# fjdf/slaMEM

Measured on AMD Instinct MI355X. Metric: MEMs/sec (and queries/sec) on 100 Mbp ref x 10 M 150 bp queries, l=20, higher is better.
Workload: dtype u32; 1 GPU; synthetic 100000000 bp reference (splitmix64 seed 42) x 10000000 reads/GPU of 150 bp, 2% substitutions, 50% reverse-complemented, -b -l 20; ref_len=100000000, reads_total=10000000, read_len=150, min_len=20, both_strands=True, parallelism=query shards x1, one GPU, no replication

## Files before the change

### include/slamem_hip.h

```cpp
#ifndef SLAMEM_HIP_H
#define SLAMEM_HIP_H

#include <stddef.h>
#include <stdint.h>

#ifdef __cplusplus
extern "C" {
#endif

#define SLAMEM_ABI_VERSION 4

enum {
    SLAMEM_OK = 0,
    SLAMEM_ERR_ARG = 1,
    SLAMEM_ERR_HIP = 2,
    SLAMEM_ERR_NOMEM = 3,
    SLAMEM_ERR_CAPACITY = 4,
    SLAMEM_ERR_FORMAT = 5,
    SLAMEM_ERR_IO = 6,
    SLAMEM_ERR_NO_DEVICE = 7
};

typedef struct slamem_index slamem_index;

// ... 69 lines not shown
    uint64_t positions;
    uint64_t enum_jobs;
    uint64_t prefilter_probes;
    uint64_t prefilter_query_loads;
    uint64_t prefilter_items;
    uint64_t items;
    uint64_t survivors;
    uint64_t mems;
    uint64_t overflow_records;
    uint64_t valid;
    uint64_t dir_sa_lines;
    uint64_t dir_group_loads;
    uint64_t dir_rec_lines;
    uint64_t dir_letters;
    uint64_t jump_lines;
    uint64_t skip_group_loads;
    uint64_t skip_probe_lines;
    uint64_t skip_attempts;
    uint64_t skips;
    uint64_t enum_row_steps;
    uint64_t enum_levels;
    uint64_t enum_wave_us;
    uint64_t state_lane_trips[11];
    uint64_t state_wave_trips[11];
    uint64_t seed_windows;
    uint64_t seed_compares;
    uint64_t seed_letter_masks;
    uint64_t seed_mems;
    uint64_t seed_strands_left;
    uint64_t seed_reads;
    uint64_t seed_query_bytes;
    uint64_t seed_left_why[7];
    uint64_t seed_once_reads;
} slamem_search_stats;

int slamem_abi_version(void);
const char *slamem_strerror(int code);
const char *slamem_last_error_message(void);
int slamem_device_count(int *count_out);
int slamem_device_warmup(int device);
int slamem_device_pci_bus_id(int device, char *out, int out_bytes);
int slamem_device_mem_info(int device, uint64_t *free_out, uint64_t *total_out);
int slamem_get_timings(slamem_timings *out);
int slamem_reset_timings(void);
int slamem_search_stats_enable(int on);
int slamem_get_search_stats(slamem_search_stats *out);
int slamem_get_search_clock(double *us_to_empty_list, double *us_tail, double *us_wave_sum);

int slamem_index_build(const char *text_host, uint32_t n, int device, slamem_index **out);
int slamem_index_build_device(const void *text_dev, uint32_t n, int device, void *stream, slamem_index **out);
int slamem_index_build_layout(const char *text_host, uint32_t n, int device, int layout, slamem_index **out);
int slamem_index_build_device_layout(const void *text_dev, uint32_t n, int device, void *stream, int layout,
                                     slamem_index **out);
int slamem_index_build_bytes(uint32_t n, int layout, uint64_t *arena_bytes_out, uint64_t *peak_bytes_out);
int slamem_index_free(slamem_index *idx);
int slamem_index_get_info(const slamem_index *idx, slamem_index_info *out);

int slamem_index_arena(const slamem_index *idx, void **arena_dev_out, uint64_t *bytes_out);
int slamem_index_export(const slamem_index *idx, void *dst_dev, uint64_t dst_bytes, void *stream);
int slamem_index_attach(void *arena_dev, uint64_t bytes, int device, slamem_index **out);
int slamem_index_adopt_arena(slamem_index *idx);
int slamem_index_save(const slamem_index *idx, const char *path);
int slamem_index_load(const char *path, int device, slamem_index **out);
int slamem_index_validate_header(const void *header, uint64_t header_bytes, uint64_t available_bytes);

enum {
// ... 190 lines not shown
```

### slamem_amd/capi.py

```python
from __future__ import annotations

import ctypes as C
import os

_HERE = os.path.dirname(os.path.abspath(__file__))
LIB_PATH = os.environ.get("SLAMEM_HIP_LIB") or os.path.join(_HERE, "csrc", "libslamem_hip.so")
SYNTH_PATH = os.path.join(_HERE, "csrc", "libslamem_synth.so")

SLAMEM_OK = 0
SLAMEM_ERR_ARG = 1
SLAMEM_ERR_HIP = 2
SLAMEM_ERR_NOMEM = 3
SLAMEM_ERR_CAPACITY = 4
SLAMEM_ERR_FORMAT = 5
SLAMEM_ERR_IO = 6
SLAMEM_ERR_NO_DEVICE = 7

ARRAY_SA, ARRAY_BWT, ARRAY_LCP, ARRAY_PSV, ARRAY_NSV = range(5)
LAYOUT_AUTO, LAYOUT_FULL, LAYOUT_COMPACT = 0, 1, 2

ABI_SYMBOLS = (
    "slamem_abi_version", "slamem_strerror", "slamem_last_error_message", "slamem_device_count",
    "slamem_get_timings", "slamem_reset_timings", "slamem_device_warmup", "slamem_device_pci_bus_id",
    "slamem_index_build", "slamem_index_build_device", "slamem_index_build_layout", "slamem_index_build_device_layout",
# ... 38 lines not shown
    _fields_ = [("text_length", C.c_uint32), ("bwt_size", C.c_uint32), ("num_n_rows", C.c_uint32),
                ("dollar_row", C.c_uint32), ("max_lcp", C.c_uint32), ("sort_rounds", C.c_uint32),
                ("arena_bytes", C.c_uint64), ("device", C.c_int32), ("owns_arena", C.c_int32),
                ("filter_k", C.c_uint32), ("layout", C.c_uint32), ("seed_k", C.c_uint32), ("reserved1", C.c_uint32)]


class SslcpStats(C.Structure):
    _fields_ = [("num_samples", C.c_uint64), ("num_oversized_lcp", C.c_uint64), ("sum_lcp", C.c_int64),
                ("max_lcp", C.c_uint32), ("pad", C.c_uint32), ("num_oversized_links", C.c_uint64),
                ("sum_link_distance", C.c_uint64), ("max_link_distance", C.c_uint64)]


class Timings(C.Structure):
    _fields_ = [("build_total_ms", C.c_float), ("build_pack_ms", C.c_float), ("build_sort_ms", C.c_float),
                ("build_bwt_ms", C.c_float), ("build_lcp_ms", C.c_float), ("build_links_ms", C.c_float),
                ("search_kernel_ms", C.c_float), ("search_total_ms", C.c_float),
                ("search_launches", C.c_uint64), ("search_kernel_ms_sum", C.c_double),
                ("prefilter_ms", C.c_float), ("k8_ms", C.c_float), ("prefilter_ms_sum", C.c_double),
                ("k8_ms_sum", C.c_double), ("seed_ms", C.c_float), ("mum_filter_ms", C.c_float), ("seed_ms_sum", C.c_double)]

    def as_dict(self):
        return {k: getattr(self, k) for k, _ in self._fields_}


class SearchStats(C.Structure):
    _fields_ = [(k, C.c_uint64) for k in (
        "fm_lines_top", "fm_lines_bottom", "rec_lines_fail", "rec_lines_pend", "rec_lines_flush", "query_loads",
        "lane_trips", "wave_trips", "positions", "enum_jobs", "prefilter_probes", "prefilter_query_loads",
        "prefilter_items", "items", "survivors", "mems", "overflow_records", "valid", "dir_sa_lines", "dir_group_loads",
        "dir_rec_lines", "dir_letters", "jump_lines", "skip_group_loads", "skip_probe_lines", "skip_attempts", "skips",
        "enum_row_steps", "enum_levels", "enum_wave_us")] + [("state_lane_trips", C.c_uint64 * 11),
                                                               ("state_wave_trips", C.c_uint64 * 11)] + [
        (k, C.c_uint64) for k in ("seed_windows", "seed_compares", "seed_letter_masks", "seed_mems", "seed_strands_left",
                                  "seed_reads", "seed_query_bytes")] + [("seed_left_why", C.c_uint64 * 7), ("seed_once_reads", C.c_uint64)]

    def as_dict(self):
        return {k: (list(getattr(self, k)) if (k.startswith("state_") or k == "seed_left_why") else int(getattr(self, k))) for k, _ in self._fields_}


_LIB = None
_SYNTH = None


def _declare(L):
    vp, u32, u64, i32 = C.c_void_p, C.c_uint32, C.c_uint64, C.c_int
    L.slamem_abi_version.restype = i32
    L.slamem_strerror.restype = C.c_char_p
    L.slamem_strerror.argtypes = [i32]
    L.slamem_last_error_message.restype = C.c_char_p
    L.slamem_device_count.argtypes = [C.POINTER(i32)]
    L.slamem_device_pci_bus_id.argtypes = [i32, C.c_char_p, i32]
    L.slamem_get_timings.argtypes = [C.POINTER(Timings)]
    L.slamem_index_build.argtypes = [C.c_char_p, u32, i32, C.POINTER(vp)]
    L.slamem_index_build_device.argtypes = [vp, u32, i32, vp, C.POINTER(vp)]
    L.slamem_index_build_layout.argtypes = [C.c_char_p, u32, i32, i32, C.POINTER(vp)]
    L.slamem_index_build_device_layout.argtypes = [vp, u32, i32, vp, i32, C.POINTER(vp)]
    L.slamem_index_build_bytes.argtypes = [u32, i32, C.POINTER(u64), C.POINTER(u64)]
    L.slamem_device_mem_info.argtypes = [i32, C.POINTER(u64), C.POINTER(u64)]
    L.slamem_index_free.argtypes = [vp]
    L.slamem_index_get_info.argtypes = [vp, C.POINTER(IndexInfo)]
    L.slamem_index_arena.argtypes = [vp, C.POINTER(vp), C.POINTER(u64)]
    L.slamem_index_export.argtypes = [vp, vp, u64, vp]
    L.slamem_index_attach.argtypes = [vp, u64, i32, C.POINTER(vp)]
    L.slamem_index_adopt_arena.argtypes = [vp]
    L.slamem_index_save.argtypes = [vp, C.c_char_p]
    L.slamem_index_load.argtypes = [C.c_char_p, i32, C.POINTER(vp)]
    L.slamem_index_validate_header.argtypes = [vp, u64, u64]
    L.slamem_search_stats_enable.argtypes = [i32]
    L.slamem_get_search_stats.argtypes = [C.POINTER(SearchStats)]
    L.slamem_get_search_clock.argtypes = [C.POINTER(C.c_double), C.POINTER(C.c_double), C.POINTER(C.c_double)]
# ... 126 lines not shown
```

### slamem_amd/csrc/mem_search.hip

```cpp
#include "common.h"
#include "prims.h"

#include <atomic>
#include <type_traits>
#include <new>
#include <stdlib.h>
#include <string.h>

namespace slamem {

struct Blk {
    uint4 a;
    uint4 b;
    uint4 c;
    uint4 d;
};

__device__ __forceinline__ uint64_t u64_of(uint32_t lo, uint32_t hi) { return ((uint64_t)hi << 32) | lo; }

__device__ __forceinline__ Blk load_blk(const FMBlock* __restrict__ fm, uint32_t bi) {
    const uint4* p = reinterpret_cast<const uint4*>(fm + bi);
    Blk k;
    k.a = p[0]; k.b = p[1]; k.c = p[2]; k.d = p[3];
    return k;
// ... 938 lines not shown
                    aoff = 0; boff = 0;
                    done = msz < L;
                }
                if (done) {
                    if (gl == 0u) A.defer.pool[segabs] = k - kbase;
                    busy = false;
                }
            }
        }
    }
#ifdef SLAMEM_DIAG_TRIPS
    if (lane == 0u) { atomicMax(A.defer.njobs + 11, dg_steps); atomicAdd(A.defer.njobs + 12, dg_steps); atomicAdd(A.defer.njobs + 13, dg_busy); }
#endif
}

__global__ void __launch_bounds__(256) k_defer_prefix(SearchArgs A) {
    const uint32_t n = *A.defer.nlist;
    for (uint32_t i = blockIdx.x * blockDim.x + threadIdx.x; i < n; i += gridDim.x * blockDim.x) {
        const uint2 e = A.defer.list[i];
        uint32_t* c = A.defer.pool + e.y;
        const uint32_t jobs = c[0], own = c[1];
        uint32_t run = 0;
        for (uint32_t s2 = 0; s2 < jobs; s2++) { const uint32_t v = c[2u + s2]; c[2u + s2] = run; run += v; }
        c[2u + jobs] = run;
        A.block_counts[e.x] = own + run;
    }
}

enum : uint32_t {
    SC_FM_TOP = 0, SC_FM_BOT, SC_REC_FAIL_LINES, SC_REC_PEND_LINES, SC_REC_FLUSH_LINES, SC_QUERY_LOADS, SC_LANE_TRIPS,
    SC_WAVE_TRIPS, SC_POSITIONS, SC_ENUM_JOBS, SC_ENUM_ROW_STEPS, SC_PF_PROBES, SC_PF_QUERY_LOADS, SC_PF_ITEMS,
    SC_DIR_SA, SC_DIR_GROUPS, SC_DIR_RECS, SC_DIR_QLOADS, SC_DIR_LETTERS, SC_JUMP_LINES,
    SC_SKIP_GROUPS, SC_SKIP_QLOADS, SC_SKIP_PROBES, SC_SKIP_OK, SC_T_FIRST, SC_T_DRAIN, SC_T_LAST, SC_T_WAVE_SUM, SC_ENUM_LEVELS, SC_T_ENUM_SUM, SC_STATE_TRIPS , SC_STATE_WAVES = SC_STATE_TRIPS + 11 ,
    SC_SEED_WINDOWS = SC_STATE_WAVES + 11, SC_SEED_COMPARES, SC_SEED_NMASKS, SC_SEED_MEMS, SC_SEED_LEFT, SC_SEED_READS, SC_SEED_QBYTES, SC_SEED_WHY , SC_SEED_ONCE = SC_SEED_WHY + 7, SC_COUNT
};
template <bool kStats>
__device__ __forceinline__ void stat_flush(unsigned long long* dst, uint32_t v) {
    if (!kStats) return;
    for (int o = 32; o > 0; o >>= 1) v += __shfl_down(v, o);
    if ((threadIdx.x & 63u) == 0u && v) atomicAdd(dst, (unsigned long long)v);
}

template <uint32_t kLanes>
__global__ void __launch_bounds__(256) k_pack_queries(SearchArgs A, bool long_only) {
    __shared__ uint8_t lut[512];
    for (uint32_t i = threadIdx.x; i < 256u; i += 256u) {
        uint32_t c = ascii_code_q(i);
        lut[i] = (uint8_t)c;
        lut[256u + i] = (uint8_t)(c >= 2u ? 7u - c : c);
    }
    __syncthreads();
    const uint32_t sub = threadIdx.x & (kLanes - 1u);
    const uint64_t count = long_only ? A.num_items : (A.work_ids ? (uint64_t)*A.work_count : A.num_items);
    const uint64_t stride = ((uint64_t)gridDim.x * blockDim.x) / kLanes;
    for (uint64_t e = ((uint64_t)blockIdx.x * blockDim.x + threadIdx.x) / kLanes; e < count; e += stride) {
    const uint64_t item = (!long_only && A.work_ids) ? (uint64_t)A.work_ids[e] : e;
    ItemDesc d;
    uint64_t pk_word;
    if (A.implicit_items) {
        if (!long_only && A.item_alive && A.item_alive[item] == 0) continue;
        d = item_of(A, item); pk_word = item_pk_of(A, item, d);
    }
    else {
        uint4 dv = *reinterpret_cast<const uint4*>(A.items + item);
        pk_word = A.item_pk[item];
        asm volatile("" : "+v"(dv.x), "+v"(dv.y), "+v"(dv.z), "+v"(dv.w), "+v"(pk_word));
        d.base = u64_of(dv.x, dv.y); d.len = dv.z; d.slice_rev = dv.w;
    }
// ... 1076 lines not shown
        unsigned long long smask[2 * R];
    };
    uint32_t flags;
    uint32_t pad[3];
};

__device__ __forceinline__ void wave_sync() {
    __builtin_amdgcn_fence(__ATOMIC_RELEASE, "wavefront");
    __builtin_amdgcn_wave_barrier();
    __builtin_amdgcn_fence(__ATOMIC_ACQUIRE, "wavefront");
}
__device__ __forceinline__ uint64_t funnel64(uint64_t lo, uint64_t hi, uint32_t sh) { return (lo >> sh) | ((hi << 1) << (63u - sh)); }
__device__ __forceinline__ uint64_t bits_below(int x) {
    const int c = x < 0 ? 0 : x > 64 ? 64 : x;
    return c == 0 ? 0ull : (~0ull >> (64 - c));
}
__device__ __forceinline__ uint64_t bits_range(int lo, int hi) { return bits_below(hi) & ~bits_below(lo); }
__device__ __forceinline__ uint32_t sel4(const uint4& v, uint32_t a) {
    const uint32_t lo = (a & 1u) ? v.y : v.x, hi = (a & 1u) ? v.w : v.z;
    return (a & 2u) ? hi : lo;
}
__device__ __forceinline__ uint32_t sel12(const uint4& b0, const uint4& b1, const uint4& b2, uint32_t e) {
    const uint32_t a = e & 3u, x0 = sel4(b0, a), x1 = sel4(b1, a), x2 = sel4(b2, a);
    return e < 4u ? x0 : e < 8u ? x1 : x2;
}
__device__ __forceinline__ uint32_t byte_tops(uint32_t m) {
    const uint32_t y = m >> 7;
    return (y | (y >> 7) | (y >> 14) | (y >> 21)) & 0xFu;
}

#ifndef SLAMEM_SEED_WAVES
#define SLAMEM_SEED_WAVES 1
#endif
template <bool kStats, uint32_t NW, uint32_t R>
__global__ void __launch_bounds__(256, SLAMEM_SEED_WAVES) k_seed_mems(SearchArgs A, uint8_t* __restrict__ alive) {
    constexpr uint32_t kMaxLen = 64u * NW;
    static_assert(R <= 32u && R * NW <= 128u, "a flag word holds a bit per read; the planes step runs in at most two passes");
    __shared__ SeedWave<NW, R> lds[4];
    const IndexView& ix = A.ix;
    const uint32_t lane = threadIdx.x & 63u, wv = threadIdx.x >> 6;
    SeedWave<NW, R>& S = lds[wv];
    const uint32_t strands = A.strands, k = ix.seed_k, L = A.min_len, s = L - k + 1u;
    const uint32_t kmask = (1u << k) - 1u;
    const uint64_t r0 = ((uint64_t)blockIdx.x * 4u + wv) * R;
    if (r0 >= (uint64_t)A.num_queries) return;
    const uint32_t nr = (uint64_t)A.num_queries - r0 < R ? (uint32_t)((uint64_t)A.num_queries - r0) : R;
    const unsigned long long below = (1ull << lane) - 1ull;
    const int64_t ulast = (int64_t)text_units(ix.n) - 1;
    uint32_t n_win = 0, n_cmp = 0, n_nm = 0, n_mem = 0;

    const uint64_t off = lane <= nr ? A.offsets[r0 + lane] : 0ull;
    constexpr uint32_t kRawChunks = R * NW * 4u + 1u, kSpecIters = (kRawChunks + 63u) / 64u;
#ifndef SLAMEM_SEED_NO_SPEC
    constexpr bool kSpec = kSpecIters <= 5u;
#else
    constexpr bool kSpec = false;
#endif
    uint4 sv[kSpec ? kSpecIters : 1u];
    uint64_t g0 = 0, len0 = 0;
    bool spec = false;
    if (kSpec) {
        const uint64_t o0 = A.offsets[0], o1 = A.offsets[1], o_end = A.offsets[A.num_queries];
        len0 = o1 - o0;
        g0 = o0 + r0 * len0;
        const uint64_t g1 = g0 + (uint64_t)nr * len0;
        spec = len0 != 0ull && len0 <= (uint64_t)kMaxLen && g1 <= o_end;
        const uint32_t gn = spec ? (uint32_t)(((g1 - 1u) >> 4) - (g0 >> 4) + 1u) : 0u;
        const uint4* src = reinterpret_cast<const uint4*>(A.qwords) + (g0 >> 4);
#pragma unroll
        for (uint32_t j = 0; j < kSpecIters; j++) {
            const uint32_t c = lane + 64u * j;
            sv[j] = c < gn ? src[c] : make_uint4(0, 0, 0, 0);
        }
    }
    const uint64_t offn = __shfl_down(off, 1);
    if (kSpec) spec = spec && __ballot(lane <= nr && off != g0 + (uint64_t)lane * len0) == 0ull;
    uint32_t len = 0, nwin = 0;
// ... 241 lines not shown
            njobs = njobs0;
        }
    };
    auto lookups = [&](uint32_t round) {
        const uint32_t step = round == 0u ? mstep : 1u;
        uint32_t cnt = 0;
        const uint32_t per = 64u >> lg_slots, wi = lane & ((1u << lg_slots) - 1u);
        const uint32_t wmod = wi - mstep * ((wi * (65536u / mstep + 1u)) >> 16);
        for (uint32_t r = 0;; r += per) {
            if (r < nr) {
                const uint32_t rr = r + (lane >> lg_slots);
                const uint32_t nw = (rr >= nr || ((S.flags >> rr) & 1u)) ? 0u : S.nwin[rr];
                const bool pred = wi < nw && (round == 0u ? wmod == 0u : wmod != 0u && ((S.expl[rr] >> wi) & 1ull) == 0ull);
                const unsigned long long pm = __ballot(pred);
                if (pred) S.ring[cnt + (uint32_t)__popcll(pm & below)] = (uint16_t)((rr << 8) | wi);
                cnt += (uint32_t)__popcll(pm);
            }
            const bool last = r >= nr;
            if (cnt >= 64u || (last && cnt != 0u)) {
                wave_sync();
                const bool act = lane < cnt;
                const uint32_t ent = act ? S.ring[lane] : 0u;
                const uint32_t over = lane + 64u < cnt ? S.ring[lane + 64u] : 0u;
                wave_sync();
                if (lane + 64u < cnt) S.ring[lane] = (uint16_t)over;
                cnt = cnt > 64u ? cnt - 64u : 0u;
                trip(ent, act, step);
            }
            if (last) break;
        }
        wave_sync();
    };

    auto compares = [&](uint32_t round) {
        const bool mark = round == 0u && mstep > 1u;
        const uint32_t ms = mstep * s;
        const uint32_t gone = S.flags;
        for (uint32_t jb = 0; jb < njobs; jb += 64u) {
            const bool listed = jb + lane < njobs;
            const uint32_t p = listed ? S.job_p[jb + lane] : 0u, xx = listed ? S.job_x[jb + lane] : 0u;
            const uint32_t os = xx & 0x7FFFu, st = (xx >> 15) & 1u, jr = xx >> 16;
            const bool has = listed && ((gone >> jr) & 1u) == 0u;
            const uint32_t Lj = S.len[jr];
            const int64_t d = (int64_t)p - (int64_t)os;
            const int64_t u0 = d >> 6;
            const uint32_t sh = (uint32_t)(d & 63);
            bool is_mem = false;
            uint32_t key = 0, ref = 0, sig = 0;
            if (has) {
                constexpr int NU = (int)NW + 1;
                int64_t ui[NU];
#pragma unroll
                for (int i = 0; i < NU; i++) { const int64_t u = u0 + i; ui[i] = u < 0 ? 0 : u > ulast ? ulast : u; }
                const uint4* T = reinterpret_cast<const uint4*>(ix.tpl);
                uint4 tu[NU], tx[NU];
#pragma unroll
                for (int i = 0; i < NU; i++) { tu[i] = T[2 * ui[i]]; tx[i] = T[2 * ui[i] + 1]; }
                uint64_t uq[NU], nu[NU];
                uint32_t anyn = 0;
#pragma unroll
                for (int i = 0; i < NU; i++) { nu[i] = u64_of(tx[i].x, tx[i].y); uq[i] = u64_of(tx[i].z, tx[i].w); anyn |= (tx[i].x | tx[i].y); }
                if (kStats && anyn) n_nm++;
                const uint64_t* R0 = S.pl[jr][st][0];
                const uint64_t* R1 = S.pl[jr][st][1];
                uint64_t mm[NW];
#pragma unroll
                for (int w = 0; w < (int)NW; w++)
                    mm[w] = (funnel64(u64_of(tu[w].x, tu[w].y), u64_of(tu[w + 1].x, tu[w + 1].y), sh) ^ R0[w]) |
                            (funnel64(u64_of(tu[w].z, tu[w].w), u64_of(tu[w + 1].z, tu[w + 1].w), sh) ^ R1[w]) | funnel64(nu[w], nu[w + 1], sh);
                if (hasn) {
                    const uint64_t* PN = S.pn[jr];
                    if (st == 0u) {
#pragma unroll
                        for (int w = 0; w < (int)NW; w++) mm[w] |= PN[w];
                    } else {
                        const uint32_t shn = kMaxLen - Lj, qn = shn >> 6, rn = shn & 63u;
#pragma unroll
                        for (int w = 0; w < (int)NW; w++) {
                            const uint32_t x = (uint32_t)w + qn;
                            const uint64_t lo64 = x < NW ? __brevll(PN[NW - 1u - x]) : 0ull, hi64 = x + 1u < NW ? __brevll(PN[NW - 2u - x]) : 0ull;
                            mm[w] |= funnel64(lo64, hi64, rn);
                        }
                    }
                }
                const int lo = d < 0 ? (int)(-d) : 0;
                const int64_t room = (int64_t)ix.n - d;
                const int hi = room < (int64_t)Lj ? (int)room : (int)Lj;
#pragma unroll
                for (int w = 0; w < (int)NW; w++) mm[w] |= ~bits_range(lo - 64 * w, hi - 64 * w);
                uint32_t a = 0, b = kMaxLen;
                bool broken = false;
#pragma unroll
                for (int w = 0; w < (int)NW; w++) {
                    const uint64_t lw = mm[w] & bits_range(0, (int)os - 64 * w);
                    if (lw) a = 64u * w + 64u - (uint32_t)__clzll((long long)lw);
                    if (mm[w] & bits_range((int)os - 64 * w, (int)(os + k) - 64 * w)) broken = true;
                }
#pragma unroll
                for (int w = (int)NW - 1; w >= 0; w--) {
                    const uint64_t hw = mm[w] & ~bits_range(0, (int)(os + k) - 64 * w);
                    if (hw) b = 64u * w + (uint32_t)__ffsll((unsigned long long)hw) - 1u;
                }
                const uint32_t af = st ? Lj - b : a, bf = st ? Lj - a : b, of = st ? Lj - k - os : os;
                bool owner;
                if (round == 0u) owner = !(of >= ms && of - ms >= af);
                else {
                    const uint32_t oa = (af + ms - 1u) / ms * ms;
                    owner = !(mstep > 1u && oa + k <= bf) && !(of >= s && of - s >= af);
                }
                if (broken) {
                    atomicOr(&S.flags, 1u << jr);
                    if (kStats) atomicAdd(A.stats + SC_SEED_WHY + 4u, 1ull);
                }
                else if (owner && b - a >= L && (strands == 2u || st == 0u)) {
                    is_mem = true; key = (a << 16) | (b - a); ref = (uint32_t)(d + (int64_t)a);
                    if (!anyn && b + kSigLetters <= kMaxLen && d + (int64_t)b + (int64_t)kSigLetters <= (int64_t)ix.n) {
                        const uint32_t wb = b >> 6, sb = b & 63u;
                        uint64_t l0 = 0, h0 = 0, l1 = 0, h1 = 0;
#pragma unroll
                        for (int w = 0; w < (int)NW; w++) {
                            const uint64_t t0 = funnel64(u64_of(tu[w].x, tu[w].y), u64_of(tu[w + 1].x, tu[w + 1].y), sh);
                            const uint64_t t1 = funnel64(u64_of(tu[w].z, tu[w].w), u64_of(tu[w + 1].z, tu[w + 1].w), sh);
                            if ((uint32_t)w == wb) { l0 = t0; l1 = t1; }
                            if ((uint32_t)w == wb + 1u) { h0 = t0; h1 = t1; }
                        }
                        sig = kSigKnown | ((uint32_t)funnel64(l0, h0, sb) & kSigMask) | (((uint32_t)funnel64(l1, h1, sb) & kSigMask) << kSigLetters);
                    }
                }
                if (mark && !broken && bf >= af + k) {
                    uint64_t uqs[NW];
#pragma unroll
                    for (int w = 0; w < (int)NW; w++) uqs[w] = funnel64(uq[w], uq[w + 1], sh);
                    unsigned long long done = 0ull;
                    for (uint32_t wi = (af + s - 1u) / s, wl = (bf - k) / s; wi <= wl; wi++) {
                        const uint32_t x = st ? Lj - k - wi * s : wi * s;
                        uint64_t word = 0ull;
#pragma unroll
                        for (int w = 0; w < (int)NW; w++) word = (x >> 6) == (uint32_t)w ? uqs[w] : word;
                        if ((word >> (x & 63u)) & 1ull) done |= 1ull << wi;
                    }
                    if (done) atomicOr(&S.expl[jr], done);
                }
            }
            if (kStats) {
                const uint32_t nh = (uint32_t)__popcll(__ballot(has));
                n_cmp += nh;
                if (mark && lane == 0u) atomicAdd(A.stats + SC_SEED_ONCE, (unsigned long long)nh);
            }
            const unsigned long long mb = __ballot(is_mem);
            if (is_mem) {
                const uint32_t at = nmems + (uint32_t)__popcll(mb & below);
                if (at < SeedWave<NW, R>::kMems) { S.mem_key[at] = key; S.mem_ref[at] = ref; S.mem_sig[at] = sig | ((2u * jr + st) << 25); }
                else { atomicOr(&S.flags, 1u << jr); if (kStats) atomicAdd(A.stats + SC_SEED_WHY + 5u, 1ull); }
            }
            nmems += (uint32_t)__popcll(mb);
        }
        wave_sync();
    };

    for (uint32_t round = 0; round < (mstep > 1u ? 2u : 1u); round++) {
        njobs = 0;
        lookups(round);
        compares(round);
    }
    };
    if (wave_hasn) search(std::true_type{}); else search(std::false_type{});
    {
        if (nmems > SeedWave<NW, R>::kMems) nmems = SeedWave<NW, R>::kMems;

        const uint32_t g0 = (uint32_t)(r0 * strands);
        auto rank_of = [&](uint32_t mi, uint32_t key, uint32_t g, uint32_t& rank, uint32_t& cnt, bool& tie) {
            rank = 0; cnt = 0; tie = false;
            for (uint32_t t2 = 0; t2 < nmems; t2++) {
                const uint32_t kk = S.mem_key[t2], gg = S.mem_sig[t2] >> 25;
                const bool same = gg == g;
                cnt += same ? 1u : 0u;
                rank += (same && kk > key) ? 1u : 0u;
                tie = tie || (same && kk == key && t2 != mi);
            }
        };
        auto tie_rank = [&](uint32_t mi, uint32_t key, uint32_t myref, uint32_t g, uint32_t sig, uint32_t& rank) -> bool {
            const uint32_t a = key >> 16, b = a + (key & 0xFFFFu);
            bool child = false;
            for (uint32_t t2 = 0; t2 < nmems; t2++) {
                const uint32_t kk = S.mem_key[t2], a2 = kk >> 16, b2 = a2 + (kk & 0xFFFFu);
                child = child || ((S.mem_sig[t2] >> 25) == g && kk != key && a2 <= a && b2 > b);
            }
            const uint32_t jr = g >> 1, st = g & 1u;
            uint32_t qb = 0;
            if (child) qb = (uint32_t)((S.pl[jr][st][0][b >> 6] >> (b & 63u)) & 1ull) | ((uint32_t)((S.pl[jr][st][1][b >> 6] >> (b & 63u)) & 1ull) << 1);
            auto letter = [&](uint32_t sg, uint32_t t) { return ((sg >> t) & 1u) | (((sg >> (t + kSigLetters)) & 1u) << 1); };
            const bool rows = ix.prec != nullptr;
            const uint32_t my_side = child && letter(sig, 0u) > qb ? 1u : 0u;
            bool bad = (sig & kSigKnown) == 0u && (child || !rows);
            for (uint32_t t2 = 0; t2 < nmems; t2++) {
                const uint32_t so = S.mem_sig[t2];
// ... 58 lines not shown
                    bool tie;
                    rank_of(mi, key, g, rank, cnt, tie);
                    const bool bad = has && tie && tie_rank(mi, key, ref, g, S.mem_sig[mi], rank);
                    if (!pass) { if (bad) atomicOr(&S.flags, 1u << (g >> 1)); }
                    else if (has) emit_mem(fl, key, ref, g, rank, cnt);
                }
                wave_sync();
            }
        }
    }
    wave_sync();
    const uint32_t fl = S.flags | wflags;
    {
        const bool isleft = lane < nr * strands && ((fl >> (strands == 2u ? lane >> 1 : lane)) & 1u) != 0u;
        if (lane < nr * strands) alive[r0 * strands + lane] = isleft ? 1 : 0;
        const unsigned long long lm = __ballot(isleft);
        if (lm != 0ull) {
            unsigned int at = 0;
            if (lane == 0u) at = atomicAdd(A.seed_left_count, (unsigned int)__popcll(lm));
            at = (unsigned int)__builtin_amdgcn_readfirstlane((int)at);
            if (isleft) A.seed_left_ids[at + (uint32_t)__popcll(lm & below)] = (uint32_t)(r0 * strands + lane);
        }
    }
    if (kStats) {
        stat_flush<kStats>(A.stats + SC_SEED_NMASKS, n_nm);
        stat_flush<kStats>(A.stats + SC_SEED_MEMS, n_mem);
        if (lane == 0u) {
            atomicAdd(A.stats + SC_SEED_WINDOWS, (unsigned long long)n_win);
            atomicAdd(A.stats + SC_SEED_COMPARES, (unsigned long long)n_cmp);
            atomicAdd(A.stats + SC_SEED_READS, (unsigned long long)nr);
            atomicAdd(A.stats + SC_SEED_QBYTES, (unsigned long long)(__builtin_amdgcn_readlane((int)(uint32_t)off, (int)nr) - __builtin_amdgcn_readlane((int)(uint32_t)off, 0)));
            atomicAdd(A.stats + SC_SEED_LEFT, (unsigned long long)(strands * (uint32_t)__popc(fl)));
            atomicAdd(A.stats + SC_SEED_WHY + 0u, (unsigned long long)__popc(wflags));
        }
    }
}

__global__ void __launch_bounds__(256) k_place_inline(const RawRow* __restrict__ inl, uint64_t stride, const uint32_t* __restrict__ counts,
                                                      const uint64_t* __restrict__ item_off, uint64_t nitems,
                                                      const uint32_t* __restrict__ sa, uint64_t capacity,
                                                      slamem_mem* __restrict__ out, const uint8_t* __restrict__ inline_valid) {
    uint64_t g = (uint64_t)blockIdx.x * blockDim.x + threadIdx.x;
    if (g >= nitems) return;
    uint32_t cnt = counts[g];
    uint64_t off = item_off[g];
    uint32_t iv = inline_valid ? inline_valid[g] : 0u;
    asm volatile("" : "+v"(cnt), "+v"(off), "+v"(iv));
    if (cnt > kInlineMems) cnt = kInlineMems;
    if (iv && cnt > iv - 1u) cnt = iv - 1u;
    if (cnt == 0u) return;
    static_assert(kInlineMems == 4, "k_place_inline is written for four inline slots");
    const RawRow* in = inl + g;
    const RawRow none = {0u, 0u, 0x80000000u};
    RawRow r0 = in[0], r1 = none, r2 = none, r3 = none;
    if (cnt > 1u) r1 = in[stride];
    if (cnt > 2u) r2 = in[2u * stride];
    if (cnt > 3u) r3 = in[3u * stride];
    asm volatile("" : "+v"(r0.row), "+v"(r0.pos), "+v"(r0.len), "+v"(r1.row), "+v"(r1.pos), "+v"(r1.len));
    asm volatile("" : "+v"(r2.row), "+v"(r2.pos), "+v"(r2.len), "+v"(r3.row), "+v"(r3.pos), "+v"(r3.len));
    uint32_t p0 = r0.row, p1 = r1.row, p2 = r2.row, p3 = r3.row;
    if (!(r0.len >> 31)) p0 = sa[r0.row];
    if (cnt > 1u && !(r1.len >> 31)) p1 = sa[r1.row];
    if (cnt > 2u && !(r2.len >> 31)) p2 = sa[r2.row];
    if (cnt > 3u && !(r3.len >> 31)) p3 = sa[r3.row];
    asm volatile("" : "+v"(p0), "+v"(p1), "+v"(p2), "+v"(p3));
    if (off < capacity) out[off] = slamem_mem{p0, r0.pos, r0.len & 0x7FFFFFFFu};
// ... 503 lines not shown

int SearchJob::prep(hipStream_t stream) {
    SLAMEM_HIP(hipSetDevice(idx->device));
    char* ws = static_cast<char*>(workspace_dev);
    unsigned long long* d_total = reinterpret_cast<unsigned long long*>(ws + w.off_total);
    uint32_t* d_counts = reinterpret_cast<uint32_t*>(ws + w.off_counts);
    prefiltered = false; timed_k8 = false; launched = true; seeded = false; rawkey_marked = false;
    (void)hipEventRecord(ev[0], stream);
    if (nitems && (match_type != 1 || mam_v3)) {
        static const bool use_filter = [] { const char* v = getenv("SLAMEM_KFILTER"); return !(v && atoi(v) == 0); }();
        seeded = seed_path;
        if (seeded) {
            uint8_t* d_alive = reinterpret_cast<uint8_t*>(ws + w.off_alive);
            if (mems_capacity && !A.skip_w && !want_stats && enum_chunks()) {
                STEP(hipMemsetAsync(ws + w.off_rawkey, 0xFF, mems_capacity * sizeof(RawKey), stream), "memset");
                rawkey_marked = true;
            }
            STEP(hipMemsetAsync(d_counts, 0, nitems * 4, stream), "memset");
            STEP(hipMemsetAsync(A.item_attempt, 0, nitems, stream), "memset");
            {
                const char* v = getenv("SLAMEM_SEED_STEP");
                A.seed_step = v && atoi(v) >= 1 && atoi(v) <= 6 ? (uint32_t)atoi(v) : 0u;
            }
            uint32_t* d_ids = reinterpret_cast<uint32_t*>(ws + w.off_workids);
            uint32_t* d_nwork = reinterpret_cast<uint32_t*>(d_total) + 8;
            A.seed_left_ids = d_ids;
            A.seed_left_count = d_nwork;
            A.seed_long_flag = reinterpret_cast<unsigned int*>(d_total) + 3;
            A.seed_wide = reinterpret_cast<unsigned int*>(d_total) + 4;
            seed_words_avg = query_bytes > (uint64_t)num_queries * kSeedMaxLenMid ? 6u : query_bytes > (uint64_t)num_queries * kSeedMaxLen ? 4u : 3u;
            const uint32_t hint = __atomic_load_n(&idx->seed_words_hint, __ATOMIC_RELAXED);
            seed_words = seed_words_avg > hint ? seed_words_avg : hint;
            const bool mid_reads = seed_words == 4u, long_reads = seed_words == 6u;
            const dim3 gs(grid_for((uint64_t)num_queries, 4 * (long_reads ? kSeedReadsLong : mid_reads ? kSeedReadsMid : kSeedReads)));
            if (long_reads) {
                if (want_stats) hipLaunchKernelGGL((k_seed_mems<true, 6, kSeedReadsLong>), gs, dim3(256), 0, stream, A, d_alive);
                else hipLaunchKernelGGL((k_seed_mems<false, 6, kSeedReadsLong>), gs, dim3(256), 0, stream, A, d_alive);
            } else if (mid_reads) {
                if (want_stats) hipLaunchKernelGGL((k_seed_mems<true, 4, kSeedReadsMid>), gs, dim3(256), 0, stream, A, d_alive);
                else hipLaunchKernelGGL((k_seed_mems<false, 4, kSeedReadsMid>), gs, dim3(256), 0, stream, A, d_alive);
            } else {
                if (want_stats) hipLaunchKernelGGL((k_seed_mems<true, 3, kSeedReads>), gs, dim3(256), 0, stream, A, d_alive);
                else hipLaunchKernelGGL((k_seed_mems<false, 3, kSeedReads>), gs, dim3(256), 0, stream, A, d_alive);
            }
            STEP(hipGetLastError(), "k_seed_mems");
            (void)hipEventRecord(ev[3], stream);
            prefiltered = true;
            A.item_alive = d_alive;
            A.work_ids = d_ids;
            A.work_count = d_nwork;
            if (use_filter && idx->view.kfilter && min_len >= idx->view.kfilter_k) {
                hipLaunchKernelGGL(k_prefilter_list, dim3(512), dim3(256), 0, stream, A, (const uint32_t*)d_ids, (const uint32_t*)d_nwork, d_alive);
                STEP(hipGetLastError(), "k_prefilter_list");
            }
        } else if (use_filter && idx->view.kfilter && min_len >= idx->view.kfilter_k) {
            uint8_t* d_alive = reinterpret_cast<uint8_t*>(ws + w.off_alive);
            if (want_stats) hipLaunchKernelGGL(k_prefilter<true>, dim3(grid_for(nitems)), dim3(256), 0, stream, A, d_alive);
            else hipLaunchKernelGGL(k_prefilter<false>, dim3(grid_for(nitems)), dim3(256), 0, stream, A, d_alive);
            STEP(hipGetLastError(), "k_prefilter");
            (void)hipEventRecord(ev[3], stream);
            prefiltered = true;
            A.item_alive = d_alive;
            STEP(hipMemsetAsync(d_counts, 0, nitems * 4, stream), "memset");
            STEP(hipMemsetAsync(A.item_attempt, 0, nitems, stream), "memset");
            uint32_t* d_ids = reinterpret_cast<uint32_t*>(ws + w.off_workids);
            uint32_t* d_nwork = reinterpret_cast<uint32_t*>(d_total) + 8;
            size_t need2 = w.select_bytes;
            STEP(select_indices_u32(ws + w.off_select, need2, d_alive, d_ids, d_nwork, nitems, stream), "select");
            A.work_ids = d_ids;
            A.work_count = d_nwork;
        }
        if (A.item_flags) STEP(hipMemsetAsync(A.item_flags, 0, nitems, stream), "memset");
        if (nitems != num_blocks) {
            static const uint32_t env_warm = [] { const char* v = getenv("SLAMEM_SLICE_WARMUP"); return v && atoi(v) > 0 ? (uint32_t)atoi(v) : kWarmUp; }();
            SliceState* d_states = reinterpret_cast<SliceState*>(ws + w.off_slicestate);
            A.item_block = reinterpret_cast<const uint32_t*>(ws + w.off_itemblock);
// ... 295 lines not shown
        if (next != hint) __atomic_store_n(hp, next, __ATOMIC_RELAXED);
    }
    if ((uint32_t)(scal[4] >> 32) != 0u) {
        set_error("slamem_find_mems_device: one work item emits 2^28 or more MEMs (a 4096-position slice against a highly "
                  "repetitive text with a small minimum length); raise min_len");
        return SLAMEM_ERR_ARG;
    }
    if (want_stats) {
        unsigned long long c[SC_COUNT];
        const uint32_t nwork = (uint32_t)scal[4];
        STEP(hipMemcpy(c, A.stats, sizeof(c), hipMemcpyDeviceToHost), "memcpy(stats)");
        slamem_search_stats& o = last_search_stats();
        memset(&o, 0, sizeof(o));
        o.fm_lines_top = c[SC_FM_TOP]; o.fm_lines_bottom = c[SC_FM_BOT];
        o.rec_lines_fail = c[SC_REC_FAIL_LINES]; o.rec_lines_pend = c[SC_REC_PEND_LINES]; o.rec_lines_flush = c[SC_REC_FLUSH_LINES];
        o.query_loads = c[SC_QUERY_LOADS]; o.lane_trips = c[SC_LANE_TRIPS]; o.wave_trips = c[SC_WAVE_TRIPS];
        o.positions = c[SC_POSITIONS]; o.enum_jobs = c[SC_ENUM_JOBS];
        o.dir_sa_lines = c[SC_DIR_SA]; o.dir_group_loads = c[SC_DIR_GROUPS]; o.dir_rec_lines = c[SC_DIR_RECS];
        o.dir_letters = c[SC_DIR_LETTERS]; o.jump_lines = c[SC_JUMP_LINES];
        o.skip_group_loads = c[SC_SKIP_GROUPS]; o.skip_probe_lines = c[SC_SKIP_PROBES]; o.skips = c[SC_SKIP_OK];
        o.skip_attempts = c[SC_SKIP_QLOADS];
        o.enum_row_steps = c[SC_ENUM_ROW_STEPS]; o.enum_levels = c[SC_ENUM_LEVELS];
        last_search_clock()[0] = (c[SC_T_DRAIN] - c[SC_T_FIRST]) / 100.0;
        last_search_clock()[1] = (c[SC_T_LAST] - c[SC_T_DRAIN]) / 100.0;
        last_search_clock()[2] = c[SC_T_WAVE_SUM] / 100.0;
        o.enum_wave_us = c[SC_T_ENUM_SUM] / 100;
        for (int q = 0; q < 11; q++) { o.state_lane_trips[q] = c[SC_STATE_TRIPS + q]; o.state_wave_trips[q] = c[SC_STATE_WAVES + q]; }
        o.prefilter_probes = c[SC_PF_PROBES]; o.prefilter_query_loads = c[SC_PF_QUERY_LOADS]; o.prefilter_items = c[SC_PF_ITEMS];
        o.seed_windows = c[SC_SEED_WINDOWS]; o.seed_compares = c[SC_SEED_COMPARES]; o.seed_letter_masks = c[SC_SEED_NMASKS];
        o.seed_mems = c[SC_SEED_MEMS]; o.seed_strands_left = c[SC_SEED_LEFT]; o.seed_reads = c[SC_SEED_READS];
        o.seed_query_bytes = c[SC_SEED_QBYTES];
        for (int q = 0; q < 7; q++) o.seed_left_why[q] = c[SC_SEED_WHY + q];
        o.seed_once_reads = c[SC_SEED_ONCE];
        o.items = nitems;
        o.survivors = prefiltered ? nwork : nitems;
        o.mems = total;
        o.overflow_records = listed;
        o.valid = match_type != 1 ? 1 : 0;
    }
    float ms = 0, ms_prep = 0, ms_k8 = 0;
    if (hipEventElapsedTime(&ms, ev[0], ev[5]) == hipSuccess) ms_prep = ms;
    if (timed_k8 && hipEventElapsedTime(&ms, ev[4], ev[1]) == hipSuccess) {
        ms_k8 = ms;
        tm.t.k8_ms = ms;
        tm.t.k8_ms_sum += ms;
    } else if (hipEventElapsedTime(&ms, ev[5], ev[1]) == hipSuccess) ms_k8 = ms;
    tm.t.search_kernel_ms = ms_prep + ms_k8;
    tm.t.search_kernel_ms_sum += ms_prep + ms_k8;
    tm.t.search_launches++;
    if (prefiltered && hipEventElapsedTime(&ms, ev[0], ev[3]) == hipSuccess) {
        if (seeded) { tm.t.seed_ms = ms; tm.t.seed_ms_sum += ms; tm.t.prefilter_ms = 0; }
        else { tm.t.prefilter_ms = ms; tm.t.prefilter_ms_sum += ms; tm.t.seed_ms = 0; }
    }
    if (hipEventElapsedTime(&ms, ev[1], ev[2]) == hipSuccess) tm.t.search_total_ms = ms_prep + ms_k8 + ms;
    aln_totals[0] = total; aln_totals[1] = 0; aln_totals[2] = 0;
    if (total > mems_capacity || listed > mems_capacity) {
        if (listed > total) total = listed;
        if (chunked) total += kK8Waves * kOvfChunk;
        aln_totals[0] = total;
        set_error("slamem_find_mems_device: %llu MEMs found, output capacity is %llu", (unsigned long long)total,
                  (unsigned long long)mems_capacity);
        return SLAMEM_ERR_CAPACITY;
    }
    tm.t.mum_filter_ms = 0;
    if (!filter) return SLAMEM_OK;
    if (hipEventElapsedTime(&ms, ev_mum[0], ev_mum[1]) == hipSuccess) tm.t.mum_filter_ms = ms;
// ... 139 lines not shown
```

Baseline: 4.959 billion MEMs/s.

## Shrink seed kernel blocks to one wave and carry partial job tails into round two

The seed-MEM kernel now launches one 64-lane wave per block instead of four, so a finished wave no longer keeps an LDS slot reserved while its block siblings are still running. In the compare step, a small leftover group of round-A jobs (fewer than 16 beyond a full 64-lane pass) is carried over and processed together with the round-B jobs instead of spending a mostly idle pass on it. Carried jobs are tagged with a high bit so they keep round-A ownership rules. New stats counters record job histograms, wave time and idle time, which adds atomics when stats are enabled.

```diff
diff --git a/include/slamem_hip.h b/include/slamem_hip.h
--- a/include/slamem_hip.h
+++ b/include/slamem_hip.h
@@ -125,6 +125,13 @@
     uint64_t seed_query_bytes;
     uint64_t seed_left_why[7];
     uint64_t seed_once_reads;
+    uint64_t seed_carried;
+    uint64_t seed_waves;
+    uint64_t seed_wave_ticks;
+    uint64_t seed_idle_ticks;
+    uint64_t seed_jobs_a[40];
+    uint64_t seed_jobs_b[40];
+    uint64_t seed_few_lane_passes[3];
 } slamem_search_stats;
 
 int slamem_abi_version(void);
diff --git a/slamem_amd/capi.py b/slamem_amd/capi.py
--- a/slamem_amd/capi.py
+++ b/slamem_amd/capi.py
@@ -94,10 +94,12 @@
         "enum_row_steps", "enum_levels", "enum_wave_us")] + [("state_lane_trips", C.c_uint64 * 11),
                                                                ("state_wave_trips", C.c_uint64 * 11)] + [
         (k, C.c_uint64) for k in ("seed_windows", "seed_compares", "seed_letter_masks", "seed_mems", "seed_strands_left",
-                                  "seed_reads", "seed_query_bytes")] + [("seed_left_why", C.c_uint64 * 7), ("seed_once_reads", C.c_uint64)]
+                                  "seed_reads", "seed_query_bytes")] + [("seed_left_why", C.c_uint64 * 7), ("seed_once_reads", C.c_uint64)] + [
+        (k, C.c_uint64) for k in ("seed_carried", "seed_waves", "seed_wave_ticks", "seed_idle_ticks")] + [
+        ("seed_jobs_a", C.c_uint64 * 40), ("seed_jobs_b", C.c_uint64 * 40), ("seed_few_lane_passes", C.c_uint64 * 3)]
 
     def as_dict(self):
-        return {k: (list(getattr(self, k)) if (k.startswith("state_") or k == "seed_left_why") else int(getattr(self, k))) for k, _ in self._fields_}
+        return {k: (list(v) if isinstance(v, C.Array) else int(v)) for k, v in ((k, getattr(self, k)) for k, _ in self._fields_)}
 
 
 _LIB = None
diff --git a/slamem_amd/csrc/mem_search.hip b/slamem_amd/csrc/mem_search.hip
--- a/slamem_amd/csrc/mem_search.hip
+++ b/slamem_amd/csrc/mem_search.hip
@@ -994,8 +994,11 @@
     SC_WAVE_TRIPS, SC_POSITIONS, SC_ENUM_JOBS, SC_ENUM_ROW_STEPS, SC_PF_PROBES, SC_PF_QUERY_LOADS, SC_PF_ITEMS,
     SC_DIR_SA, SC_DIR_GROUPS, SC_DIR_RECS, SC_DIR_QLOADS, SC_DIR_LETTERS, SC_JUMP_LINES,
     SC_SKIP_GROUPS, SC_SKIP_QLOADS, SC_SKIP_PROBES, SC_SKIP_OK, SC_T_FIRST, SC_T_DRAIN, SC_T_LAST, SC_T_WAVE_SUM, SC_ENUM_LEVELS, SC_T_ENUM_SUM, SC_STATE_TRIPS , SC_STATE_WAVES = SC_STATE_TRIPS + 11 ,
-    SC_SEED_WINDOWS = SC_STATE_WAVES + 11, SC_SEED_COMPARES, SC_SEED_NMASKS, SC_SEED_MEMS, SC_SEED_LEFT, SC_SEED_READS, SC_SEED_QBYTES, SC_SEED_WHY , SC_SEED_ONCE = SC_SEED_WHY + 7, SC_COUNT
+    SC_SEED_WINDOWS = SC_STATE_WAVES + 11, SC_SEED_COMPARES, SC_SEED_NMASKS, SC_SEED_MEMS, SC_SEED_LEFT, SC_SEED_READS, SC_SEED_QBYTES, SC_SEED_WHY , SC_SEED_ONCE = SC_SEED_WHY + 7,
+    SC_SEED_CARRIED, SC_SEED_T_WAVES, SC_SEED_T_IDLE, SC_SEED_NWAVES, SC_SEED_JOBS_A ,
+    SC_SEED_JOBS_B = SC_SEED_JOBS_A + 40 , SC_SEED_FEW = SC_SEED_JOBS_B + 40 , SC_COUNT = SC_SEED_FEW + 3
 };
+constexpr uint32_t kSeedJobBins = 40;
 template <bool kStats>
 __device__ __forceinline__ void stat_flush(unsigned long long* dst, uint32_t v) {
     if (!kStats) return;
@@ -2138,17 +2141,34 @@
 #ifndef SLAMEM_SEED_WAVES
 #define SLAMEM_SEED_WAVES 1
 #endif
+#ifndef SLAMEM_SEED_BLOCK_WAVES
+#define SLAMEM_SEED_BLOCK_WAVES 1
+#endif
+constexpr uint32_t kSeedBlockWaves = SLAMEM_SEED_BLOCK_WAVES;
+#ifndef SLAMEM_SEED_CARRY
+#define SLAMEM_SEED_CARRY 16
+#endif
+constexpr uint32_t kSeedCarry = SLAMEM_SEED_CARRY;
+static_assert(kSeedCarry <= 64u, "a carried tail is less than one pass");
+constexpr uint32_t kJobRoundA = 1u << 31;
 template <bool kStats, uint32_t NW, uint32_t R>
-__global__ void __launch_bounds__(256, SLAMEM_SEED_WAVES) k_seed_mems(SearchArgs A, uint8_t* __restrict__ alive) {
+__global__ void __launch_bounds__(64 * SLAMEM_SEED_BLOCK_WAVES, SLAMEM_SEED_WAVES) k_seed_mems(SearchArgs A, uint8_t* __restrict__ alive) {
     constexpr uint32_t kMaxLen = 64u * NW;
     static_assert(R <= 32u && R * NW <= 128u, "a flag word holds a bit per read; the planes step runs in at most two passes");
-    __shared__ SeedWave<NW, R> lds[4];
+    __shared__ SeedWave<NW, R> lds[kSeedBlockWaves];
     const IndexView& ix = A.ix;
-    const uint32_t lane = threadIdx.x & 63u, wv = threadIdx.x >> 6;
+    const uint32_t lane = threadIdx.x & 63u, wv = kSeedBlockWaves > 1u ? threadIdx.x >> 6 : 0u;
     SeedWave<NW, R>& S = lds[wv];
+    __shared__ unsigned long long blk_end_sum, blk_end_max;
+    __shared__ uint32_t blk_done;
+    if (kStats && kSeedBlockWaves > 1u) {
+        if (threadIdx.x == 0u) { blk_end_sum = 0ull; blk_end_max = 0ull; blk_done = 0u; }
+        __syncthreads();
+    }
+    const unsigned long long t_wave0 = kStats ? wall_clock64() : 0ull;
     const uint32_t strands = A.strands, k = ix.seed_k, L = A.min_len, s = L - k + 1u;
     const uint32_t kmask = (1u << k) - 1u;
-    const uint64_t r0 = ((uint64_t)blockIdx.x * 4u + wv) * R;
+    const uint64_t r0 = ((uint64_t)blockIdx.x * kSeedBlockWaves + wv) * R;
     if (r0 >= (uint64_t)A.num_queries) return;
     const uint32_t nr = (uint64_t)A.num_queries - r0 < R ? (uint32_t)((uint64_t)A.num_queries - r0) : R;
     const unsigned long long below = (1ull << lane) - 1ull;
@@ -2456,15 +2476,26 @@
         wave_sync();
     };
 
-    auto compares = [&](uint32_t round) {
+    auto compares = [&](uint32_t round) -> uint32_t {
         const bool mark = round == 0u && mstep > 1u;
         const uint32_t ms = mstep * s;
         const uint32_t gone = S.flags;
-        for (uint32_t jb = 0; jb < njobs; jb += 64u) {
-            const bool listed = jb + lane < njobs;
+        if (kStats && lane == 0u) {
+            const uint32_t bin = njobs / 8u < kSeedJobBins - 1u ? njobs / 8u : kSeedJobBins - 1u, tail = njobs & 63u;
+            atomicAdd(A.stats + (round == 0u ? SC_SEED_JOBS_A : SC_SEED_JOBS_B) + bin, 1ull);
+            if (mark && njobs > 64u && tail != 0u)
+                for (uint32_t q = 0; q < 3u; q++)
+                    if (tail < 8u * (q + 1u)) atomicAdd(A.stats + SC_SEED_FEW + q, 1ull);
+        }
+        uint32_t carry = 0;
+        if (kSeedCarry != 0u && mark && njobs > 64u && (njobs & 63u) != 0u && (njobs & 63u) < kSeedCarry) carry = njobs & 63u;
+        const uint32_t ncmp = njobs - carry;
+        for (uint32_t jb = 0; jb < ncmp; jb += 64u) {
+            const bool listed = jb + lane < ncmp;
             const uint32_t p = listed ? S.job_p[jb + lane] : 0u, xx = listed ? S.job_x[jb + lane] : 0u;
-            const uint32_t os = xx & 0x7FFFu, st = (xx >> 15) & 1u, jr = xx >> 16;
-            const bool has = listed && ((gone >> jr) & 1u) == 0u;
+            const uint32_t os = xx & 0x7FFFu, st = (xx >> 15) & 1u, jr = (xx >> 16) & 0x1Fu;
+            const bool ja = kSeedCarry != 0u ? (round == 0u || (xx & kJobRoundA) != 0u) : round == 0u;
+            const bool has = listed && ((gone >> jr) & 1u) == 0u && !(kSeedCarry != 0u && round != 0u && ja && strands == 1u && st != 0u);
             const uint32_t Lj = S.len[jr];
             const int64_t d = (int64_t)p - (int64_t)os;
             const int64_t u0 = d >> 6;
@@ -2527,7 +2558,7 @@
                 }
                 const uint32_t af = st ? Lj - b : a, bf = st ? Lj - a : b, of = st ? Lj - k - os : os;
                 bool owner;
-                if (round == 0u) owner = !(of >= ms && of - ms >= af);
+                if (ja) owner = !(of >= ms && of - ms >= af);
                 else {
                     const uint32_t oa = (af + ms - 1u) / ms * ms;
                     owner = !(mstep > 1u && oa + k <= bf) && !(of >= s && of - s >= af);
@@ -2579,13 +2610,18 @@
             }
             nmems += (uint32_t)__popcll(mb);
         }
+        uint32_t cp = 0, cx = 0;
+        if (lane < carry) { cp = S.job_p[ncmp + lane]; cx = S.job_x[ncmp + lane] | kJobRoundA; }
         wave_sync();
+        if (lane < carry) { S.job_p[lane] = cp; S.job_x[lane] = cx; }
+        if (kStats && carry && lane == 0u) atomicAdd(A.stats + SC_SEED_CARRIED, (unsigned long long)carry);
+        return carry;
     };
 
-    for (uint32_t round = 0; round < (mstep > 1u ? 2u : 1u); round++) {
-        njobs = 0;
+    for (uint32_t round = 0, carried = 0; round < (mstep > 1u ? 2u : 1u); round++) {
+        njobs = carried;
         lookups(round);
-        compares(round);
+        carried = compares(round);
     }
     };
     if (wave_hasn) search(std::true_type{}); else search(std::false_type{});
@@ -2710,6 +2746,20 @@
             atomicAdd(A.stats + SC_SEED_QBYTES, (unsigned long long)(__builtin_amdgcn_readlane((int)(uint32_t)off, (int)nr) - __builtin_amdgcn_readlane((int)(uint32_t)off, 0)));
             atomicAdd(A.stats + SC_SEED_LEFT, (unsigned long long)(strands * (uint32_t)__popc(fl)));
             atomicAdd(A.stats + SC_SEED_WHY + 0u, (unsigned long long)__popc(wflags));
+            const unsigned long long t_end = wall_clock64();
+            atomicAdd(A.stats + SC_SEED_T_WAVES, t_end - t_wave0);
+            atomicAdd(A.stats + SC_SEED_NWAVES, 1ull);
+            if (kSeedBlockWaves > 1u) {
+                const uint64_t rb = (uint64_t)blockIdx.x * kSeedBlockWaves * R, left = (uint64_t)A.num_queries - rb;
+                const uint32_t waves = left >= (uint64_t)kSeedBlockWaves * R ? kSeedBlockWaves : (uint32_t)((left + R - 1u) / R);
+                atomicAdd(&blk_end_sum, t_end);
+                atomicMax(&blk_end_max, t_end);
+                __threadfence_block();
+                if (atomicAdd(&blk_done, 1u) + 1u == waves) {
+                    __threadfence_block();
+                    atomicAdd(A.stats + SC_SEED_T_IDLE, atomicMax(&blk_end_max, 0ull) * waves - atomicAdd(&blk_end_sum, 0ull));
+                }
+            }
         }
     }
 }
@@ -3279,16 +3329,16 @@
             const uint32_t hint = __atomic_load_n(&idx->seed_words_hint, __ATOMIC_RELAXED);
             seed_words = seed_words_avg > hint ? seed_words_avg : hint;
             const bool mid_reads = seed_words == 4u, long_reads = seed_words == 6u;
-            const dim3 gs(grid_for((uint64_t)num_queries, 4 * (long_reads ? kSeedReadsLong : mid_reads ? kSeedReadsMid : kSeedReads)));
+            const dim3 gs(grid_for((uint64_t)num_queries, kSeedBlockWaves * (long_reads ? kSeedReadsLong : mid_reads ? kSeedReadsMid : kSeedReads))), bs(64u * kSeedBlockWaves);
             if (long_reads) {
-                if (want_stats) hipLaunchKernelGGL((k_seed_mems<true, 6, kSeedReadsLong>), gs, dim3(256), 0, stream, A, d_alive);
-                else hipLaunchKernelGGL((k_seed_mems<false, 6, kSeedReadsLong>), gs, dim3(256), 0, stream, A, d_alive);
+                if (want_stats) hipLaunchKernelGGL((k_seed_mems<true, 6, kSeedReadsLong>), gs, bs, 0, stream, A, d_alive);
+                else hipLaunchKernelGGL((k_seed_mems<false, 6, kSeedReadsLong>), gs, bs, 0, stream, A, d_alive);
             } else if (mid_reads) {
-                if (want_stats) hipLaunchKernelGGL((k_seed_mems<true, 4, kSeedReadsMid>), gs, dim3(256), 0, stream, A, d_alive);
-                else hipLaunchKernelGGL((k_seed_mems<false, 4, kSeedReadsMid>), gs, dim3(256), 0, stream, A, d_alive);
+                if (want_stats) hipLaunchKernelGGL((k_seed_mems<true, 4, kSeedReadsMid>), gs, bs, 0, stream, A, d_alive);
+                else hipLaunchKernelGGL((k_seed_mems<false, 4, kSeedReadsMid>), gs, bs, 0, stream, A, d_alive);
             } else {
-                if (want_stats) hipLaunchKernelGGL((k_seed_mems<true, 3, kSeedReads>), gs, dim3(256), 0, stream, A, d_alive);
-                else hipLaunchKernelGGL((k_seed_mems<false, 3, kSeedReads>), gs, dim3(256), 0, stream, A, d_alive);
+                if (want_stats) hipLaunchKernelGGL((k_seed_mems<true, 3, kSeedReads>), gs, bs, 0, stream, A, d_alive);
+                else hipLaunchKernelGGL((k_seed_mems<false, 3, kSeedReads>), gs, bs, 0, stream, A, d_alive);
             }
             STEP(hipGetLastError(), "k_seed_mems");
             (void)hipEventRecord(ev[3], stream);
@@ -3650,6 +3700,11 @@
         o.seed_query_bytes = c[SC_SEED_QBYTES];
         for (int q = 0; q < 7; q++) o.seed_left_why[q] = c[SC_SEED_WHY + q];
         o.seed_once_reads = c[SC_SEED_ONCE];
+        o.seed_carried = c[SC_SEED_CARRIED]; o.seed_waves = c[SC_SEED_NWAVES];
+        o.seed_wave_ticks = c[SC_SEED_T_WAVES]; o.seed_idle_ticks = c[SC_SEED_T_IDLE];
+        static_assert(sizeof(o.seed_jobs_a) / sizeof(o.seed_jobs_a[0]) == kSeedJobBins, "the bins of the header");
+        for (uint32_t q = 0; q < kSeedJobBins; q++) { o.seed_jobs_a[q] = c[SC_SEED_JOBS_A + q]; o.seed_jobs_b[q] = c[SC_SEED_JOBS_B + q]; }
+        for (int q = 0; q < 3; q++) o.seed_few_lane_passes[q] = c[SC_SEED_FEW + q];
         o.items = nitems;
         o.survivors = prefiltered ? nwork : nitems;
         o.mems = total;
```

Result: slower. 4.645 billion MEMs/s (-6.3%).
